# sriram-0311/MC-SLAM

Measured on AMD Instinct MI355X. Metric: multi-cam frames/sec (4-cam 1280x720 @2000 kpts/cam, extract + intra-rig match), higher is better.
Workload: dtype u8; 1 GPU; 4-cam rig 1280x720, 2000 kpts/cam, extract + all-pairs intra-rig match (configs[1]); slots=4, frames_per_launch=128, cameras=4, nfeatures=2000

## Files before the change

### mc-slam_amd/csrc/mcorb_kernels.hip

```cpp
#include <hip/hip_runtime.h>
#include <stdint.h>
#include <string.h>
#include <vector>

#include "mcorb_common.h"
#include "mcorb_device.h"
#include "mcorb_kernels.h"

namespace mcorb {

constexpr int kResizeRows = kResizeTileH;

template <int NF>
__global__ __launch_bounds__(256) void k_resize(uint8_t *__restrict__ pyr, Geom g, int level,
                                                const ResizeTap *__restrict__ tabs, int srcPitch, int srcRows)
{
    extern __shared__ __attribute__((aligned(16))) uint8_t win[];
    const LevelGeom &D = g.lv[level];
    const LevelGeom &S = g.lv[level - 1];
    const int img = blockIdx.z;
    uint8_t *base = pyr + (size_t)img * g.imgBytes;
    const int tid = threadIdx.x;
    const int bx0 = blockIdx.x * 256, by0 = blockIdx.y * kResizeRows;
    const int bx1 = min(bx0 + 255, D.w - 1), by1 = min(by0 + kResizeRows - 1, D.h - 1);
    const int sx0 = tabs[D.xtab + bx0].s0 & ~15, sx1 = tabs[D.xtab + bx1].s1;
    const int sy0 = tabs[D.ytab + by0].s0, sy1 = tabs[D.ytab + by1].s1;
    const int nq = ((sx1 - sx0) >> 4) + 1, nr = sy1 - sy0 + 1;
    const int wave = wave_uniform(tid >> 6);
    const int wy0 = by0 + wave * (kResizeRows / 4);
    uint2 ytap;
    {
        const int l = tid & 63;
        const int dy = min(wy0 + (l < kResizeRows / 4 ? l : 0), D.h - 1);
        ytap = *reinterpret_cast<const uint2 *>(tabs + D.ytab + dy);
    }
    const int dx4 = bx0 + (tid & 63) * 4;
    const int dxc = min(dx4, ((D.w + 3) & ~3) - 4);
    const uint4 t01 = *reinterpret_cast<const uint4 *>(tabs + D.xtab + dxc);
    const uint4 t23 = *reinterpret_cast<const uint4 *>(tabs + D.xtab + dxc + 2);
    {
        const uint8_t *sp = base + S.off + (size_t)sy0 * S.pitch + sx0;
        uint4 *w128 = reinterpret_cast<uint4 *>(win);
        const int pq = srcPitch >> 4;
        const float rcp_pq = 1.0f / (float)pq;
        if constexpr (NF > 0) {
            uint4 v[NF];
            bool ok[NF];
#pragma unroll
            for (int k = 0; k < NF; k++) {
                const int i = tid + 256 * k, ic = min(i, nr * pq - 1);
                const int r = (int)(((float)ic + 0.5f) * rcp_pq), q = ic - r * pq;
                ok[k] = i < nr * pq && q < nq;
                v[k] = *reinterpret_cast<const uint4 *>(sp + (size_t)r * S.pitch + 16 * min(q, nq - 1));
            }
            const int spare = (srcPitch >> 4) * srcRows;
#pragma unroll
            for (int k = 0; k < NF; k++) w128[ok[k] ? tid + 256 * k : spare] = v[k];
        } else {
            for (int i = tid; i < nr * pq; i += 256) {
                const int r = (int)(((float)i + 0.5f) * rcp_pq), q = i - r * pq;
                if (q < nq) w128[i] = *reinterpret_cast<const uint4 *>(sp + (size_t)r * S.pitch + 16 * q);
            }
        }
    }
    __syncthreads();
    asm volatile("" ::"v"(ytap.x), "v"(ytap.y), "v"(t01.x), "v"(t01.y), "v"(t01.z), "v"(t01.w), "v"(t23.x), "v"(t23.y), "v"(t23.z), "v"(t23.w));
    if (dx4 >= D.w) return;
    const uint32_t tw[8] = {t01.x, t01.y, t01.z, t01.w, t23.x, t23.y, t23.z, t23.w};
    int s0[4], s1[4], a0[4], a1[4];
#pragma unroll
    for (int k = 0; k < 4; k++) {
        s0[k] = (int)(tw[2 * k] & 0xffff) - sx0;
        s1[k] = (int)(tw[2 * k] >> 16) - sx0;
        a0[k] = (int)(short)(tw[2 * k + 1] & 0xffff);
        a1[k] = (int)(short)(tw[2 * k + 1] >> 16);
    }
    const uint32_t mask = dx4 + 4 > D.w ? 0xffffffffu >> (8 * (dx4 + 4 - D.w)) : 0xffffffffu;
    int rowA = -1, rowB = -1;
    uint32_t HA[4], HB[4];
    const uint32_t ldsWin = (uint32_t)(uintptr_t)(__attribute__((address_space(3))) void *)win;
    uint32_t sb[4];
#pragma unroll
    for (int k = 0; k < 4; k++) sb[k] = ldsWin + (uint32_t)s0[k];
    auto hrow = [&](int sr, uint32_t *Hout) {
        const uint32_t ro = (uint32_t)__mul24(sr - sy0, srcPitch);
        const uint32_t ad0 = sb[0] + ro, ad1 = sb[1] + ro, ad2 = sb[2] + ro, ad3 = sb[3] + ro;
        uint32_t x0, x1, x2, x3, x4, x5, x6, x7;
        asm volatile("ds_read_u8 %0, %8\n\tds_read_u8 %1, %8 offset:1\n\t"
                     "ds_read_u8 %2, %9\n\tds_read_u8 %3, %9 offset:1\n\t"
                     "ds_read_u8 %4, %10\n\tds_read_u8 %5, %10 offset:1\n\t"
                     "ds_read_u8 %6, %11\n\tds_read_u8 %7, %11 offset:1\n\t"
                     "s_waitcnt lgkmcnt(0)"
                     : "=&v"(x0), "=&v"(x1), "=&v"(x2), "=&v"(x3), "=&v"(x4), "=&v"(x5), "=&v"(x6), "=&v"(x7)
                     : "v"(ad0), "v"(ad1), "v"(ad2), "v"(ad3)
                     : "memory");
        Hout[0] = (__umul24(x0, (uint32_t)a0[0]) + __umul24(x1, (uint32_t)a1[0])) >> 4;
        Hout[1] = (__umul24(x2, (uint32_t)a0[1]) + __umul24(x3, (uint32_t)a1[1])) >> 4;
        Hout[2] = (__umul24(x4, (uint32_t)a0[2]) + __umul24(x5, (uint32_t)a1[2])) >> 4;
        Hout[3] = (__umul24(x6, (uint32_t)a0[3]) + __umul24(x7, (uint32_t)a1[3])) >> 4;
    };
#pragma unroll
    for (int rr = 0; rr < kResizeRows / 4; rr++) {
        const int dy = wy0 + rr;
        if (dy >= D.h) break;
        const uint32_t ys = (uint32_t)__builtin_amdgcn_readlane((int)ytap.x, rr), yc = (uint32_t)__builtin_amdgcn_readlane((int)ytap.y, rr);
        const int r0 = (int)(ys & 0xffff), r1 = (int)(ys >> 16);
        if (r0 != rowA) {
            if (r0 == rowB) {
#pragma unroll
                for (int k = 0; k < 4; k++) HA[k] = HB[k];
            } else {
                hrow(r0, HA);
            }
            rowA = r0;
        }
        if (r1 != rowB) {
            if (r1 == rowA) {
#pragma unroll
                for (int k = 0; k < 4; k++) HB[k] = HA[k];
            } else {
                hrow(r1, HB);
            }
            rowB = r1;
        }
        const uint32_t b0 = yc & 0xffff, b1 = yc >> 16;
        uint32_t p0[4], p1[4];
#pragma unroll
        for (int k = 0; k < 4; k++) {
            p0[k] = __umul24(b0, HA[k]) + 0x20000u;
            p1[k] = __umul24(b1, HB[k]);
        }
        uint32_t t01v, t23v;
        asm("v_add_u32_sdwa %0, %1, %2 dst_sel:DWORD dst_unused:UNUSED_PAD src0_sel:WORD_1 src1_sel:WORD_1" : "=v"(t01v) : "v"(p0[0]), "v"(p1[0]));
        asm("v_add_u32_sdwa %0, %1, %2 dst_sel:WORD_1 dst_unused:UNUSED_PRESERVE src0_sel:WORD_1 src1_sel:WORD_1" : "+v"(t01v) : "v"(p0[1]), "v"(p1[1]));
        asm("v_add_u32_sdwa %0, %1, %2 dst_sel:DWORD dst_unused:UNUSED_PAD src0_sel:WORD_1 src1_sel:WORD_1" : "=v"(t23v) : "v"(p0[2]), "v"(p1[2]));
        asm("v_add_u32_sdwa %0, %1, %2 dst_sel:WORD_1 dst_unused:UNUSED_PRESERVE src0_sel:WORD_1 src1_sel:WORD_1" : "+v"(t23v) : "v"(p0[3]), "v"(p1[3]));
        const u16x2 s01 = __builtin_bit_cast(u16x2, t01v) >> (unsigned short)2, s23 = __builtin_bit_cast(u16x2, t23v) >> (unsigned short)2;
        const uint32_t out = __builtin_amdgcn_perm(__builtin_bit_cast(uint32_t, s23), __builtin_bit_cast(uint32_t, s01), 0x06040200u);
        *reinterpret_cast<uint32_t *>(base + D.off + (size_t)dy * D.pitch + dx4) = out & mask;
    }
}


struct FastCell {
    int on;
    int cell;
    int ph;
    int wi, hi;
    int rows;
    int g0, ng;
    int R;
    float rcp_ng;
    uint32_t headMask, tailMask;
    uint32_t org;
    const uint8_t *src;
    int pitch;
};

constexpr int kFastCellRecDw = 8;
__device__ __forceinline__ void fast_cell_setup(const uint8_t *pyr, const Geom &g, int img, int cell, const uint32_t *__restrict__ rec, FastCell &C)
{
    const uint4 r = *reinterpret_cast<const uint4 *>(rec + (size_t)cell * kFastCellRecDw);
    const uint2 r4 = *reinterpret_cast<const uint2 *>(rec + (size_t)cell * kFastCellRecDw + 4);
    C.cell = cell;
    C.src = pyr + (size_t)img * g.imgBytes + r.x;
    C.org = r.y;
    C.pitch = (int)r.z;
    C.rows = (int)(r.w & 0xff);
    C.wi = (int)((r.w >> 8) & 0xff);
    C.hi = (int)((r.w >> 16) & 0xff);
    C.on = (int)((r.w >> 24) & 1);
    C.ph = (int)((r.w >> 25) & 3);
    C.g0 = (int)(r4.x & 0xff);
    C.ng = (int)((r4.x >> 8) & 0xff);
    C.R = (int)(r4.x >> 16);
    C.rcp_ng = __uint_as_float(r4.y);
    const uint2 r6 = *reinterpret_cast<const uint2 *>(rec + (size_t)cell * kFastCellRecDw + 6);
    C.headMask = r6.x;
    C.tailMask = r6.y;
}

int fast_cell_table(const Geom &g, std::vector<uint32_t> &tab)
{
    const int off = (int)tab.size();
    tab.resize(tab.size() + (size_t)g.cells * kFastCellRecDw, 0u);
    for (int level = 0; level < g.nlevels; level++) {
        const LevelGeom &L = g.lv[level];
        for (int cl = 0; cl < L.nCols * L.nRows; cl++) {
            const int ci = cl / L.nCols, cj = cl - ci * L.nCols;
            const int iniY = kMinBorder + ci * L.hCell;
            int maxY = iniY + L.hCell + 6;
            const int iniX = kMinBorder + cj * L.wCell;
            int maxX = iniX + L.wCell + 6;
            const bool skip = (iniY >= L.maxBorderY - 3) || (iniX >= L.maxBorderX - 6);
            if (maxY > L.maxBorderY) maxY = L.maxBorderY;
            if (maxX > L.maxBorderX) maxX = L.maxBorderX;
            const int cols = maxX - iniX, rows = maxY - iniY;
            const int wi = cols - 6, hi = rows - 6;
            const int ph = iniX & 3, g0 = (ph + 3) >> 2;
            const bool on = !(skip || wi <= 0 || hi <= 0);
            const int ng = on ? ((ph + 2 + wi) >> 2) - g0 + 1 : 1;
            uint32_t *r = tab.data() + off + (size_t)(L.cell0 + cl) * kFastCellRecDw;
            r[0] = on ? (uint32_t)(L.off + (size_t)iniY * L.pitch + (iniX - ph)) : 0u;
            r[1] = ((uint32_t)(ci * L.hCell) << 20) + ((uint32_t)(cj * L.wCell - ph) << 8);
            r[2] = (uint32_t)L.pitch;
            r[3] = on ? ((uint32_t)rows | ((uint32_t)wi << 8) | ((uint32_t)hi << 16) | (1u << 24) | ((uint32_t)ph << 25)) : 0u;
            r[4] = (uint32_t)g0 | ((uint32_t)ng << 8) | ((uint32_t)(64 / ng) << 16);
            const float rcp = 1.0f / (float)ng;
            uint32_t bits;
            memcpy(&bits, &rcp, 4);
            r[5] = bits;
            auto pxmask = [&](int G) {
                static const uint32_t bit[4] = {1u << 15, 1u, 1u << 31, 1u << 16};
                uint32_t m = 0;
                for (int j = 0; j < 4; j++) {
                    const int x = 4 * G + j - (ph + 3);
                    if (x >= 0 && x < wi) m |= bit[j];
                }
                return m;
            };
            r[6] = on ? pxmask(g0) : 0u;
            r[7] = on ? pxmask(g0 + ng - 1) : 0u;
        }
    }
    return off;
}

constexpr int kFastListCap = 768;

#define EMAX __builtin_elementwise_max
#define EMIN __builtin_elementwise_min
struct FastLane {
    int off0;
    uint32_t vmask;
};
template <int TP>
__device__ __forceinline__ FastLane fast_lane_setup(const FastCell &C, int lane)
{
    FastLane L;
    const int r = (int)(((float)lane + 0.5f) * C.rcp_ng);
    const int gi = lane - r * C.ng;
    const bool act = r < C.R;
    L.off0 = act ? (3 + r) * TP + 4 * (C.g0 + gi) : 3 * TP + 4 * C.g0;
    uint32_t m = 0x80018001u;
    m = gi == 0 ? m & C.headMask : m;
    m = gi == C.ng - 1 ? m & C.tailMask : m;
    L.vmask = act ? m : 0u;
    return L;
}

template <int TP>
__device__ __forceinline__ int fast_pass1(const uint8_t *tile, uint32_t *glist, const FastCell &C, int T, int lane, int &row0, int gcap,
                                          const FastLane &L)
{
    const u16x2 Tev = u16x2{(unsigned short)T, (unsigned short)T};
    const u16x2 Tod = u16x2{(unsigned short)(256 * T + 255), (unsigned short)(256 * T + 255)};
    int nG = 0;
    auto trip = [&](int rb, bool tail) {
        int off = L.off0 + rb * TP;
        bool in = true;
        if (tail) {
            in = (int)(((float)lane + 0.5f) * C.rcp_ng) + rb < C.hi;
            off = in ? off : 3 * TP + 4 * C.g0;
        }
        const uint32_t *p = reinterpret_cast<const uint32_t *>(tile + off);
        const uint32_t Cc = p[0], Cl = p[-1], Cr = p[1], Up = p[-3 * (TP / 4)], Dn = p[3 * (TP / 4)];
        const uint32_t Lf = __builtin_amdgcn_alignbyte(Cc, Cl, 1);
        const uint32_t Rt = __builtin_amdgcn_alignbyte(Cr, Cc, 3);
#define U16(X) __builtin_bit_cast(u16x2, (uint32_t)(X))
#define S16(X) __builtin_bit_cast(s16x2, (uint32_t)(X))
        const u16x2 hO = EMIN(EMAX(U16(Up), U16(Dn)), EMAX(U16(Lf), U16(Rt)));
        const u16x2 lO = EMAX(EMIN(U16(Up), U16(Dn)), EMIN(U16(Lf), U16(Rt)));
        const u16x2 hOm = U16(__builtin_bit_cast(uint32_t, hO) & 0xff00ff00u), lOm = U16(__builtin_bit_cast(uint32_t, lO) & 0xff00ff00u);
        const u16x2 vO = U16(Cc & 0xff00ff00u);
        const u16x2 wO = EMAX(__builtin_elementwise_sub_sat(hOm, vO), __builtin_elementwise_sub_sat(vO, lOm));
        const uint32_t zO = __builtin_bit_cast(uint32_t, __builtin_elementwise_sub_sat(wO, Tod));
        const s16x2 vE = S16(Cc & 0x00ff00ffu), uE = S16(Up & 0x00ff00ffu), dE = S16(Dn & 0x00ff00ffu);
        const s16x2 lE = S16(Lf & 0x00ff00ffu), rE = S16(Rt & 0x00ff00ffu);
        const s16x2 wE = EMAX(EMIN(EMAX(uE, dE), EMAX(lE, rE)) - vE, vE - EMAX(EMIN(uE, dE), EMIN(lE, rE)));
        const uint32_t sE = __builtin_bit_cast(uint32_t, __builtin_bit_cast(s16x2, Tev) - wE);
#undef U16
#undef S16
        const uint32_t M = ((sE & 0x80008000u) | (zO & 0x00010001u)) & L.vmask;
        const bool c = M != 0 && in;
        const unsigned long long b = __builtin_amdgcn_ballot_w64(c);
        if (c) glist[lane_rank(b, nG)] = M | ((uint32_t)off >> 1);
        nG += __popcll(b);
    };
    int rb = row0;
    for (; rb + C.R <= C.hi && nG + 64 <= gcap; rb += C.R) trip(rb, false);
    if (rb < C.hi && rb + C.R > C.hi && nG + 64 <= gcap) {
        trip(rb, true);
        rb += C.R;
    }
    row0 = rb;
    return nG;
}

__device__ __forceinline__ int fast_expand(const uint32_t *glist, uint16_t *work, int nG, int lane)
{
    int nA = 0;
    for (int i0 = 0; i0 < nG; i0 += 64) {
        const bool in = i0 + lane < nG;
        const uint32_t E = in ? glist[i0 + lane] : 0u;
        const uint32_t m = E & 0x80018001u;
        const int n1 = in ? __popc(m) - 1 : 0;
        const unsigned long long b0 = __builtin_amdgcn_ballot_w64((n1 & 1) != 0), b1 = __builtin_amdgcn_ballot_w64(n1 >= 2);
        int o = nA + lane + lane_rank(b0) + 2 * lane_rank(b1);
        const uint32_t off = (E & 0x3ffeu) << 1;
        asm volatile("" ::: "memory");
        if (m & 0x8000u) work[o++] = (uint16_t)off;
        if (m & 0x1u) work[o++] = (uint16_t)(off + 1);
        if (m & 0x80000000u) work[o++] = (uint16_t)(off + 2);
        if (m & 0x10000u) work[o++] = (uint16_t)(off + 3);
        const int cnt = min(nG - i0, 64);
        nA += cnt + __popcll(b0) + 2 * __popcll(b1);
        asm volatile("" ::: "memory");
    }
    return nA;
}

template <int TP>
__device__ __forceinline__ int fast_arc_score(const uint8_t *tile, int pos)
{
    int lo = pos - (3 * TP + 3);
    asm volatile("" : "+v"(lo));
    const uint8_t *c = tile + lo + (3 * TP + 3);
    u16x2 X[8];
    X[0] = u16x2{c[3 * TP], c[-3 * TP]};          X[1] = u16x2{c[3 * TP + 1], c[-3 * TP - 1]};
    X[2] = u16x2{c[2 * TP + 2], c[-2 * TP - 2]};  X[3] = u16x2{c[TP + 3], c[-TP - 3]};
    X[4] = u16x2{c[3], c[-3]};                    X[5] = u16x2{c[-TP + 3], c[TP - 3]};
    X[6] = u16x2{c[-2 * TP + 2], c[2 * TP - 2]};  X[7] = u16x2{c[-3 * TP + 1], c[3 * TP - 1]};
    const uint32_t v = c[0];
    u16x2 Sn[8], Sx[8], Pn[8], Px[8];
    Sn[7] = Sx[7] = X[7];
    Pn[0] = Px[0] = X[0];
#pragma unroll
    for (int i = 6; i >= 1; i--) { Sn[i] = EMIN(X[i], Sn[i + 1]); Sx[i] = EMAX(X[i], Sx[i + 1]); }
#pragma unroll
    for (int i = 1; i < 8; i++) { Pn[i] = EMIN(X[i], Pn[i - 1]); Px[i] = EMAX(X[i], Px[i - 1]); }
    Sn[0] = Pn[7]; Sx[0] = Px[7];
    u16x2 bn, bx;
#pragma unroll
    for (int k = 0; k < 8; k++) {
        const u16x2 wn = EMIN(Sn[k], __builtin_shufflevector(Pn[k], Pn[k], 1, 0));
        const u16x2 wx = EMAX(Sx[k], __builtin_shufflevector(Px[k], Px[k], 1, 0));
        bn = k ? EMAX(bn, wn) : wn;
        bx = k ? EMIN(bx, wx) : wx;
    }
    const int Mx = max((int)bn.x, (int)bn.y), Mn = min((int)bx.x, (int)bx.y);
    const int a = max(Mx - (int)v, (int)v - Mn);
    return a < 0 ? 0 : a;
}
#undef EMAX
#undef EMIN

template <int TP>
__global__ __launch_bounds__(64) void k_fast_cells(const uint8_t *__restrict__ pyr, Geom g, int iniTh, int minTh,
                                                   int tileB, int scB, int cap, const uint32_t *__restrict__ cellRec,
                                                   uint32_t *__restrict__ cell_kp, int *__restrict__ cell_cnt)
{
    extern __shared__ __attribute__((aligned(16))) uint8_t lds[];
    constexpr int NQ = TP / 16;
    uint8_t *tile = lds + 16;
    uint8_t *sc = tile + tileB + 16;
    uint8_t *sc2 = sc - 2 * TP;
    uint16_t *work = reinterpret_cast<uint16_t *>(sc + scB + 16);
    uint32_t *glist = reinterpret_cast<uint32_t *>(work + cap / 2);
    const int gcap = cap >> 2;
    struct __attribute__((packed, aligned(4))) Chunk { uint32_t a, b, c, d; };

    const int lane = threadIdx.x;
    const int img = blockIdx.y;
    FastCell C;
    fast_cell_setup(pyr, g, img, wave_uniform(xcd_remap(blockIdx.x, gridDim.x)), cellRec, C);
    int *out_cnt = cell_cnt + (size_t)img * g.cells + C.cell;
    if (!C.on) {
        if (lane == 0) *out_cnt = 0;
        return;
    }

    FastLane FL;
    for (int r = lane; r < C.rows; r += 64) {
        Chunk ch[NQ];
#pragma unroll
        for (int q = 0; q < NQ; q++) ch[q] = *reinterpret_cast<const Chunk *>(C.src + (size_t)r * C.pitch + 16 * q);
        uint4 *dst = reinterpret_cast<uint4 *>(tile + r * TP);
#pragma unroll
        for (int q = 0; q < NQ; q++) dst[q] = uint4{ch[q].a, ch[q].b, ch[q].c, ch[q].d};
    }
    {
        uint4 *s128 = reinterpret_cast<uint4 *>(sc);
        for (int i = lane; i < scB / 16; i += 64) s128[i] = uint4{0, 0, 0, 0};
        FL = fast_lane_setup<TP>(C, lane);
    }
    __syncthreads();

    uint32_t *dst = cell_kp + ((size_t)img * g.cells + C.cell) * g.cellCap;
    int total = 0;
    auto score = [&](int nA, int T) {
        for (int i = lane; i < nA; i += 64) {
            const int pos = work[i];
            const int a = fast_arc_score<TP>(tile, pos);
            sc2[pos] = (uint8_t)(a > T ? a : 0);
        }
    };
    auto nms = [&](int nA) {
        for (int i0 = 0; i0 < nA; i0 += 64) {
            const int i = i0 + lane;
            const int pos = i < nA ? (int)work[i] : 3 * TP;
            int lo = pos - (TP + 1);
            asm volatile("" : "+v"(lo));
            const uint8_t *s = sc2 + lo + (TP + 1);
            const uint32_t a = s[0];
            const uint32_t n = max(max(max((uint32_t)s[1], (uint32_t)s[-1]), max((uint32_t)s[-TP - 1], (uint32_t)s[-TP])),
                                   max(max((uint32_t)s[-TP + 1], (uint32_t)s[TP - 1]), max((uint32_t)s[TP], (uint32_t)s[TP + 1])));
            const bool keep = a > n;
            const unsigned long long b = __builtin_amdgcn_ballot_w64(keep);
            if (keep) {
                const int o = lane_rank(b, total);
                const int yy = (int)(((float)pos + 0.5f) * (1.0f / (float)TP)), xx = __mul24(yy, -TP) + pos;
                if (o < g.cellCap) dst[o] = C.org + ((uint32_t)yy << 20) + ((uint32_t)xx << 8) + (a - 1);
            }
            total += __popcll(b);
        }
    };
    int T = iniTh;
#pragma unroll 1
    for (int attempt = 0; attempt < 2; attempt++) {
        int row0 = 0, sweep = 0;
#pragma unroll 1
        for (;;) {
            const bool whole = row0 == 0;
            const int nG = fast_pass1<TP>(tile, glist, C, T, lane, row0, gcap, FL);
            __syncthreads();
            const int nA = fast_expand(glist, work, nG, lane);
            __syncthreads();
            if (sweep == 0) {
                score(nA, T);
                __syncthreads();
            }
            if (sweep == 1 || (whole && row0 >= C.hi)) nms(nA);
            if (row0 >= C.hi) {
                if (sweep == 1 || whole) break;
                sweep = 1;
                row0 = 0;
            }
            __syncthreads();
        }
        if (total || T == minTh) break;
        T = minTh;
        __syncthreads();
    }
    if (lane == 0) *out_cnt = total;
}

constexpr int kCompactCopies = 4;
template <int kCompactWaves>
__device__ __forceinline__ int block_exclusive_scan(int v, int *wsum, int *total)
{
    const int lane = threadIdx.x & 63, wave = threadIdx.x >> 6;
    int s = v;
#pragma unroll
    for (int o = 1; o < 64; o <<= 1) {
        const int t = __shfl_up(s, o);
        if (lane >= o) s += t;
    }
    if (lane == 63) wsum[wave] = s;
    __syncthreads();
    if (wave == 0) {
        const int w = lane < kCompactWaves ? wsum[lane] : 0;
        int t = w;
#pragma unroll
        for (int o = 1; o < kCompactWaves; o <<= 1) {
            const int u = __shfl_up(t, o);
            if (lane >= o) t += u;
        }
        if (lane < kCompactWaves) wsum[lane] = t - w;
        if (lane == kCompactWaves - 1) *total = t;
    }
    __syncthreads();
    return wsum[wave] + s - v;
}

template <int kCompactWG, int kCompactCells, int NC>
__global__ __launch_bounds__(kCompactWG, 8) void k_compact(const uint32_t *__restrict__ cell_kp, const int *__restrict__ cell_cnt,
                                                        Geom g, const uint16_t *__restrict__ lut, uint32_t *__restrict__ sorted_dev,
                                                        uint32_t *__restrict__ cand, int *__restrict__ tbl,
                                                        int *__restrict__ overflow, int bktCap, int cellsCap)
{
    extern __shared__ __attribute__((aligned(16))) int sh[];
    int *hist = sh;
    uint32_t *bkey = reinterpret_cast<uint32_t *>(hist + NC * bktCap);
    uint16_t *cnts = reinterpret_cast<uint16_t *>(hist + 2 * NC * bktCap);
    constexpr int kCompactWaves = kCompactWG / 64;
    __shared__ int wsum[kCompactWaves];
    __shared__ int s_tot, s_base, s_nz;
    const int tid = threadIdx.x, lane = tid & 63, wave = tid >> 6;
    const int level = blockIdx.y, img = blockIdx.x;
    const LevelGeom &L = g.lv[level];
    const int nc = L.nCols * L.nRows;
    const int *cnt = cell_cnt + (size_t)img * g.cells;
    const int cap = g.cellCap;
    const int B = L.nBuckets;
    const int W0 = L.maxBorderX - kMinBorder, H0 = L.maxBorderY - kMinBorder;
    uint16_t *tx = cnts + cellsCap, *ty = tx + W0;

    int s = 0, t = 0, over = 0;
    for (int c = tid; c < L.cell0; c += kCompactWG) { const int v = cnt[c]; s += v < cap ? v : cap; }
    for (int c = tid; c < nc; c += kCompactWG) {
        int v = cnt[L.cell0 + c];
        if (v > cap) { v = cap; over = 1; }
        cnts[c] = (uint16_t)v;
        t += v;
    }
    for (int c = nc + tid; c < min(nc + 2 * kCompactCells, cellsCap); c += kCompactWG) cnts[c] = 0;
    for (int i = tid; i < W0 + H0; i += kCompactWG) tx[i] = lut[L.lutx + i];
    (void)block_exclusive_scan<kCompactWaves>(s, wsum, &s_base);
    (void)block_exclusive_scan<kCompactWaves>(t, wsum, &s_tot);
    const int base = s_base, T = s_tot;
    for (int b = tid; b < NC * (B + 1); b += kCompactWG) { hist[b] = 0; bkey[b] = 0; }
    int *tb = tbl + (size_t)img * tbl_ints(g.bucketTotal);
    if (tid == 0) {
        s_nz = 0;
        tb[kTblLvlOff + level] = base;
        if (level == g.nlevels - 1) tb[kTblLvlOff + g.nlevels] = base + T;
        if (base + T > g.candCap) over = 1;
    }
    if (over) atomicOr(overflow, 1);
    __syncthreads();

    const uint32_t *src = cell_kp + ((size_t)img * g.cells + L.cell0) * cap;
    const int wave_u = wave_uniform(wave);
    auto walk = [&](auto &&fn) {
        static_assert(kCompactCells == 8 || kCompactCells == 4 || kCompactCells == 2, "the counts are read as one 4-, 8- or 16-byte word");
        constexpr int step = kCompactWaves * kCompactCells;
        const int ncUp = (nc + kCompactCells - 1) & ~(kCompactCells - 1);
        auto load = [&](int c0, int *n, uint32_t *p) {
            if constexpr (kCompactCells == 8) {
                const uint4 q = *reinterpret_cast<const uint4 *>(cnts + c0);
                n[0] = q.x & 0xffff; n[1] = q.x >> 16; n[2] = q.y & 0xffff; n[3] = q.y >> 16;
                n[4] = q.z & 0xffff; n[5] = q.z >> 16; n[6] = q.w & 0xffff; n[7] = q.w >> 16;
            } else if constexpr (kCompactCells == 4) {
                const uint2 q = *reinterpret_cast<const uint2 *>(cnts + c0);
                n[0] = q.x & 0xffff; n[1] = q.x >> 16; n[2] = q.y & 0xffff; n[3] = q.y >> 16;
            } else {
                const uint32_t q = *reinterpret_cast<const uint32_t *>(cnts + c0);
                n[0] = q & 0xffff; n[1] = q >> 16;
            }
#pragma unroll
            for (int u = 0; u < kCompactCells; u++) {
                const uint32_t *cb = src + (size_t)min(c0 + u, nc - 1) * cap;
                p[u] = cb[min(lane, max(n[u], 1) - 1)];
            }
        };
        auto run = [&](int c0, const int *n, const uint32_t *p) {
            int big = 0;
#pragma unroll
            for (int u = 0; u < kCompactCells; u++) {
                big |= n[u];
                if (lane < n[u]) fn(p[u], (c0 + u) * cap + lane);
            }
            if (big > 64) {
#pragma unroll
                for (int u = 0; u < kCompactCells; u++)
                    for (int k = lane + 64; k < n[u]; k += 64) fn(src[(size_t)(c0 + u) * cap + k], (c0 + u) * cap + k);
            }
        };
        int c0 = wave_u * kCompactCells;
        if (c0 >= nc) return;
        int nA[kCompactCells], nB[kCompactCells];
        uint32_t pA[kCompactCells], pB[kCompactCells];
        load(c0, nA, pA);
        while (true) {
            load(min(c0 + step, ncUp), nB, pB);
            run(c0, nA, pA);
            c0 += step;
            if (c0 >= nc) break;
            load(min(c0 + step, ncUp), nA, pA);
            run(c0, nB, pB);
            c0 += step;
            if (c0 >= nc) break;
        }
    };
    walk([&](uint32_t p, int order) {
        const uint32_t code = (uint32_t)tx[cand_x(p)] | (uint32_t)ty[cand_y(p)];
        const uint32_t key = ((uint32_t)cand_resp(p) << 23) | (uint32_t)(kPickOrderMask - order);
        const int slot = (int)code * NC + (lane & (NC - 1));
        atomicAdd(&hist[slot], 1);
        atomicMax(&bkey[slot], key);
    });
    __syncthreads();
    {
        const int bper = (B + kCompactWG - 1) / kCompactWG;
        const int b0 = tid * bper;
        int bs = 0, nzl = 0;
        for (int k = 0; k < bper; k++)
            if (b0 + k < B) {
                int v = 0;
#pragma unroll
                for (int c = 0; c < NC; c++) v += hist[(b0 + k) * NC + c];
                bs += v;
                nzl += v > 0;
            }
        if (nzl) atomicAdd(&s_nz, nzl);
        int brun = block_exclusive_scan<kCompactWaves>(bs, wsum, &s_tot);
        for (int k = 0; k < bper; k++) {
            if (b0 + k < B) {
#pragma unroll
                for (int c = 0; c < NC; c++) { const int v = hist[(b0 + k) * NC + c]; hist[(b0 + k) * NC + c] = brun; brun += v; }
            }
        }
        if (tid == 0) hist[B * NC] = T;
    }
    __syncthreads();
    int *bs_out = tb + kTblHead + L.bucket0;
    for (int b = tid; b <= B; b += kCompactWG) bs_out[b] = hist[b * NC];
    __syncthreads();
    uint32_t *sd = sorted_dev + (size_t)img * g.candCap + base;
    const int room = g.candCap - base;
    walk([&](uint32_t p, int) {
        const uint32_t code = (uint32_t)tx[cand_x(p)] | (uint32_t)ty[cand_y(p)];
        const int slot = atomicAdd(&hist[(int)code * NC + (lane & (NC - 1))], 1);
        if (slot < room) sd[slot] = p;
    });
    __syncthreads();
    uint2 *bb_out = reinterpret_cast<uint2 *>(tb + tbl_win_off(g.bucketTotal)) + L.bucket0;
    for (int b = tid; b < B; b += kCompactWG) {
        uint32_t k = 0;
#pragma unroll
        for (int c = 0; c < NC; c++) k = max(k, bkey[b * NC + c]);
        bb_out[b] = uint2{k, k ? src[kPickOrderMask - (k & (uint32_t)kPickOrderMask)] : 0u};
    }
    bool ship = s_nz < L.quota;
    if (ship && base + T > g.hostCandCap) {
        ship = false;
        if (tid == 0) atomicOr(overflow, 1);
    }
    if (tid == 0) tb[kTblShipped + level] = ship ? 1 : 0;
    if (ship) {
        uint32_t *dst = cand + (size_t)img * g.hostCandCap + base;
        for (int i = tid; i < T; i += kCompactWG) dst[i] = sd[i];
    }
}

template <int B>
__device__ __forceinline__ uint32_t gauss_window(const uint32_t (&D)[4])
{
    constexpr int q = B >> 2, sh = B & 3;
    if constexpr (sh == 0) return D[q];
    else return __builtin_amdgcn_alignbyte(D[q + 1], D[q], sh);
}
template <int SH>
__device__ __forceinline__ void gauss_hsum4(const uint32_t (&D)[4], uint32_t (&h)[4])
{
    constexpr uint32_t T1 = 0x38302212u, T2 = 0x00122230u;
    h[0] = __builtin_amdgcn_udot4(gauss_window<SH + 4>(D), T2, __builtin_amdgcn_udot4(gauss_window<SH>(D), T1, 0u, false), false);
    h[1] = __builtin_amdgcn_udot4(gauss_window<SH + 5>(D), T2, __builtin_amdgcn_udot4(gauss_window<SH + 1>(D), T1, 0u, false), false);
    h[2] = __builtin_amdgcn_udot4(gauss_window<SH + 6>(D), T2, __builtin_amdgcn_udot4(gauss_window<SH + 2>(D), T1, 0u, false), false);
    h[3] = __builtin_amdgcn_udot4(gauss_window<SH + 7>(D), T2, __builtin_amdgcn_udot4(gauss_window<SH + 3>(D), T1, 0u, false), false);
}
__device__ __forceinline__ uint4 gauss_pair4(const uint32_t (&h0)[4], const uint32_t (&h1)[4])
{
    return uint4{__builtin_amdgcn_perm(h1[0], h0[0], 0x05040100u), __builtin_amdgcn_perm(h1[1], h0[1], 0x05040100u),
                 __builtin_amdgcn_perm(h1[2], h0[2], 0x05040100u), __builtin_amdgcn_perm(h1[3], h0[3], 0x05040100u)};
}
__device__ __forceinline__ uint32_t gauss_vrow4(const uint32_t (&P)[5][4], int k)
{
    const int tap[9] = {0, 18, 34, 48, 56, 48, 34, 18, 0};
    const int q = k >> 1, o = 1 - (k & 1);
    uint32_t acc[4];
#pragma unroll
    for (int j = 0; j < 4; j++) {
        uint32_t a = 32768u;
#pragma unroll
        for (int i = 0; i < 4; i++)
            a = __builtin_amdgcn_udot2(__builtin_bit_cast(u16x2, P[q + i][j]), u16x2{(unsigned short)tap[2 * i + o], (unsigned short)tap[2 * i + o + 1]}, a, false);
        acc[j] = a;
    }
    return __builtin_amdgcn_perm(acc[1], acc[0], 0x0c0c0602u) | __builtin_amdgcn_perm(acc[3], acc[2], 0x06020c0cu);
}

__global__ __launch_bounds__(256) void k_blur(const uint8_t *__restrict__ pyr, uint8_t *__restrict__ blur, Geom g)
{
    constexpr int TW = kBlurTW, TH = kBlurTH;
    constexpr int ID = TW / 4 + 8, A0 = 3;
    constexpr int NP = (TH + 6) / 2;
    __shared__ __attribute__((aligned(16))) uint32_t in32[(TH + 6) * ID];
    __shared__ __attribute__((aligned(16))) uint32_t hp[NP * TW];
    const int tid = threadIdx.x;
    const int img = blockIdx.y;
    const int tile = xcd_remap(blockIdx.x, gridDim.x);
    int level = 0;
#pragma unroll 1
    for (int l = 1; l < g.nlevels; l++)
        if (tile >= g.lv[l].tile0) level = l;
    const LevelGeom &L = g.lv[level];
    const int t = tile - L.tile0;
    const int ty = t / L.tilesX, tx = t - ty * L.tilesX;
    const int x0 = tx * TW, y0 = ty * TH;
    const uint8_t *plane = pyr + (size_t)img * g.imgBytes + L.off;

    if (x0 >= 4 && x0 + TW + 4 <= L.w && y0 >= 3 && y0 + TH + 3 <= L.h) {
        constexpr int QR = TW / 16;
        constexpr int NQ = ((TH + 6) * QR + 255) / 256;
        const uint8_t *src = plane + (size_t)(y0 - 3) * L.pitch + x0;
        uint4 v[NQ];
#pragma unroll
        for (int k = 0; k < NQ; k++) {
            const int i = tid + 256 * k;
            const int r = i / QR, q = i - r * QR;
            v[k] = i < (TH + 6) * QR ? *reinterpret_cast<const uint4 *>(src + (size_t)r * L.pitch + 16 * q) : uint4{0, 0, 0, 0};
        }
        uint32_t ap = 0;
        const int ar = tid >> 1, aside = tid & 1;
        if (tid < 2 * (TH + 6)) ap = *reinterpret_cast<const uint32_t *>(src + (size_t)ar * L.pitch + (aside ? TW : -4));
#pragma unroll
        for (int k = 0; k < NQ; k++) {
            const int i = tid + 256 * k;
            const int r = i / QR, q = i - r * QR;
            if (i < (TH + 6) * QR) *reinterpret_cast<uint4 *>(in32 + r * ID + A0 + 1 + 4 * q) = v[k];
        }
        if (tid < 2 * (TH + 6)) in32[ar * ID + A0 + (aside ? TW / 4 + 1 : 0)] = ap;
    } else {
        constexpr int QR = TW / 16;
        constexpr int NQ = ((TH + 6) * QR + 255) / 256;
        auto src_row = [&](int r) {
            int sy = reflect101(y0 + r - 3, L.h);
            sy = sy < 0 ? 0 : (sy >= L.h ? L.h - 1 : sy);
            return plane + (size_t)sy * L.pitch + x0;
        };
        uint4 v[NQ];
#pragma unroll
        for (int k = 0; k < NQ; k++) {
            const int i = tid + 256 * k;
            const int r = i / QR, q = i - r * QR;
            v[k] = i < (TH + 6) * QR ? *reinterpret_cast<const uint4 *>(src_row(r) + 16 * q) : uint4{0, 0, 0, 0};
        }
        uint32_t ap = 0;
        const int ar = tid >> 1, aside = tid & 1;
        if (tid < 2 * (TH + 6) && (aside || x0 > 0)) ap = *reinterpret_cast<const uint32_t *>(src_row(ar) + (aside ? TW : -4));
#pragma unroll
        for (int k = 0; k < NQ; k++) {
            const int i = tid + 256 * k;
            const int r = i / QR, q = i - r * QR;
// ... 730 lines not shown
```

Measured before the change: 40490 frames/s.

## Rework FAST cell kernel with raw LDS addressing, score-map reuse and corner compaction

```diff
diff --git a/mc-slam_amd/csrc/mcorb_kernels.hip b/mc-slam_amd/csrc/mcorb_kernels.hip
--- a/mc-slam_amd/csrc/mcorb_kernels.hip
+++ b/mc-slam_amd/csrc/mcorb_kernels.hip
@@ -231,40 +231,57 @@
 #define EMAX __builtin_elementwise_max
 #define EMIN __builtin_elementwise_min
 struct FastLane {
-    int off0;
+    uint32_t G0;
     uint32_t vmask;
+    int r;
 };
+typedef __attribute__((address_space(3))) uint8_t lds_byte;
+__device__ __forceinline__ uint32_t lds_addr(const void *p) { return (uint32_t)(uintptr_t)(const lds_byte *)p; }
+template <typename T>
+__device__ __forceinline__ T lds_ld(uint32_t a) { return *(const __attribute__((address_space(3))) T *)(uintptr_t)a; }
+template <typename T>
+__device__ __forceinline__ void lds_st(uint32_t a, T v) { *(__attribute__((address_space(3))) T *)(uintptr_t)a = v; }
+
 template <int TP>
-__device__ __forceinline__ FastLane fast_lane_setup(const FastCell &C, int lane)
+__device__ __forceinline__ FastLane fast_lane_setup(const FastCell &C, int lane, uint32_t tileA)
 {
     FastLane L;
     const int r = (int)(((float)lane + 0.5f) * C.rcp_ng);
     const int gi = lane - r * C.ng;
     const bool act = r < C.R;
-    L.off0 = act ? (3 + r) * TP + 4 * (C.g0 + gi) : 3 * TP + 4 * C.g0;
+    L.G0 = tileA - 4 + (act ? r * TP + 4 * (C.g0 + gi) : 4 * C.g0);
     uint32_t m = 0x80018001u;
     m = gi == 0 ? m & C.headMask : m;
     m = gi == C.ng - 1 ? m & C.tailMask : m;
     L.vmask = act ? m : 0u;
+    L.r = r;
     return L;
 }
 
-template <int TP>
-__device__ __forceinline__ int fast_pass1(const uint8_t *tile, uint32_t *glist, const FastCell &C, int T, int lane, int &row0, int gcap,
-                                          const FastLane &L)
+template <int TP, bool FROM_MAP>
+__device__ __forceinline__ int fast_pass1(uint32_t tileA, uint32_t glistA, const FastCell &C, int T, int lane, int &row0, int gcap,
+                                          const FastLane &L, uint32_t scD)
 {
     const u16x2 Tev = u16x2{(unsigned short)T, (unsigned short)T};
     const u16x2 Tod = u16x2{(unsigned short)(256 * T + 255), (unsigned short)(256 * T + 255)};
-    int nG = 0;
-    auto trip = [&](int rb, bool tail) {
-        int off = L.off0 + rb * TP;
-        bool in = true;
-        if (tail) {
-            in = (int)(((float)lane + 0.5f) * C.rcp_ng) + rb < C.hi;
-            off = in ? off : 3 * TP + 4 * C.g0;
-        }
-        const uint32_t *p = reinterpret_cast<const uint32_t *>(tile + off);
-        const uint32_t Cc = p[0], Cl = p[-1], Cr = p[1], Up = p[-3 * (TP / 4)], Dn = p[3 * (TP / 4)];
+    uint32_t slot = glistA;
+    const uint32_t slotMax = glistA + 4 * (gcap - 64);
+    auto emit = [&](uint32_t G, uint32_t M, bool in) {
+        const bool c = M != 0 && in;
+        const unsigned long long b = __builtin_amdgcn_ballot_w64(c);
+        asm volatile("" : "+s"(slot));
+        if (c) lds_st<uint32_t>(slot + 4 * lane_rank(b), M | G);
+        slot += 4 * __popcll(b);
+    };
+    auto trip = [&](uint32_t G, bool in) {
+        if constexpr (FROM_MAP) {
+            const uint32_t sc4 = lds_ld<uint32_t>(G + scD);
+            const uint32_t nz = ((sc4 & 0x7f7f7f7fu) + 0x7f7f7f7fu) | sc4;
+            emit(G, (((nz & 0x00800080u) << 8) | ((nz >> 15) & 0x00010001u)) & L.vmask, in);
+            return;
+        }
+        const uint32_t Up = lds_ld<uint32_t>(G + 4), Dn = lds_ld<uint32_t>(G + 6 * TP + 4);
+        const uint32_t Cl = lds_ld<uint32_t>(G + 3 * TP), Cc = lds_ld<uint32_t>(G + 3 * TP + 4), Cr = lds_ld<uint32_t>(G + 3 * TP + 8);
         const uint32_t Lf = __builtin_amdgcn_alignbyte(Cc, Cl, 1);
         const uint32_t Rt = __builtin_amdgcn_alignbyte(Cr, Cc, 3);
 #define U16(X) __builtin_bit_cast(u16x2, (uint32_t)(X))
@@ -281,38 +298,43 @@
         const uint32_t sE = __builtin_bit_cast(uint32_t, __builtin_bit_cast(s16x2, Tev) - wE);
 #undef U16
 #undef S16
-        const uint32_t M = ((sE & 0x80008000u) | (zO & 0x00010001u)) & L.vmask;
-        const bool c = M != 0 && in;
-        const unsigned long long b = __builtin_amdgcn_ballot_w64(c);
-        if (c) glist[lane_rank(b, nG)] = M | ((uint32_t)off >> 1);
-        nG += __popcll(b);
+        uint32_t sel = (sE & 0x80008000u) | (zO & ~0x80008000u);
+        asm volatile("" : "+v"(sel));
+        emit(G, sel & L.vmask, in);
     };
     int rb = row0;
-    for (; rb + C.R <= C.hi && nG + 64 <= gcap; rb += C.R) trip(rb, false);
-    if (rb < C.hi && rb + C.R > C.hi && nG + 64 <= gcap) {
-        trip(rb, true);
+    uint32_t G = L.G0 + rb * TP;
+    for (; rb + C.R <= C.hi && slot <= slotMax; rb += C.R, G += C.R * TP) {
+        asm volatile("" : "+v"(G));
+        trip(G, true);
+    }
+    if (rb < C.hi && rb + C.R > C.hi && slot <= slotMax) {
+        const bool in = L.r + rb < C.hi;
+        uint32_t Gt = in ? G : tileA - 4 + 4 * C.g0;
+        asm volatile("" : "+v"(Gt));
+        trip(Gt, in);
         rb += C.R;
     }
     row0 = rb;
-    return nG;
-}
-
-__device__ __forceinline__ int fast_expand(const uint32_t *glist, uint16_t *work, int nG, int lane)
+    return (int)(slot - glistA) >> 2;
+}
+
+__device__ __forceinline__ int fast_expand(uint32_t glistA, uint32_t workA, int nG, int lane)
 {
     int nA = 0;
     for (int i0 = 0; i0 < nG; i0 += 64) {
         const bool in = i0 + lane < nG;
-        const uint32_t E = in ? glist[i0 + lane] : 0u;
+        const uint32_t E = in ? lds_ld<uint32_t>(glistA + 4 * (i0 + lane)) : 0u;
         const uint32_t m = E & 0x80018001u;
         const int n1 = in ? __popc(m) - 1 : 0;
         const unsigned long long b0 = __builtin_amdgcn_ballot_w64((n1 & 1) != 0), b1 = __builtin_amdgcn_ballot_w64(n1 >= 2);
-        int o = nA + lane + lane_rank(b0) + 2 * lane_rank(b1);
-        const uint32_t off = (E & 0x3ffeu) << 1;
+        uint32_t o = (workA + 2 * nA) + 2 * (lane_rank(b0, lane) + 2 * lane_rank(b1));
+        const uint32_t G = E & 0x7ffcu;
         asm volatile("" ::: "memory");
-        if (m & 0x8000u) work[o++] = (uint16_t)off;
-        if (m & 0x1u) work[o++] = (uint16_t)(off + 1);
-        if (m & 0x80000000u) work[o++] = (uint16_t)(off + 2);
-        if (m & 0x10000u) work[o++] = (uint16_t)(off + 3);
+        if ((int16_t)E < 0) { lds_st<uint16_t>(o, (uint16_t)G); o += 2; }
+        if (m & 0x1u) { lds_st<uint16_t>(o, (uint16_t)(G + 1)); o += 2; }
+        if (m & 0x80000000u) { lds_st<uint16_t>(o, (uint16_t)(G + 2)); o += 2; }
+        if (m & 0x10000u) lds_st<uint16_t>(o, (uint16_t)(G + 3));
         const int cnt = min(nG - i0, 64);
         nA += cnt + __popcll(b0) + 2 * __popcll(b1);
         asm volatile("" ::: "memory");
@@ -321,17 +343,15 @@
 }
 
 template <int TP>
-__device__ __forceinline__ int fast_arc_score(const uint8_t *tile, int pos)
-{
-    int lo = pos - (3 * TP + 3);
-    asm volatile("" : "+v"(lo));
-    const uint8_t *c = tile + lo + (3 * TP + 3);
+__device__ __forceinline__ int fast_arc_score(uint32_t W)
+{
+    auto px = [&](int dx, int dy) { return (unsigned short)lds_ld<uint8_t>(W + 1 + (3 + dy) * TP + (3 + dx)); };
     u16x2 X[8];
-    X[0] = u16x2{c[3 * TP], c[-3 * TP]};          X[1] = u16x2{c[3 * TP + 1], c[-3 * TP - 1]};
-    X[2] = u16x2{c[2 * TP + 2], c[-2 * TP - 2]};  X[3] = u16x2{c[TP + 3], c[-TP - 3]};
-    X[4] = u16x2{c[3], c[-3]};                    X[5] = u16x2{c[-TP + 3], c[TP - 3]};
-    X[6] = u16x2{c[-2 * TP + 2], c[2 * TP - 2]};  X[7] = u16x2{c[-3 * TP + 1], c[3 * TP - 1]};
-    const uint32_t v = c[0];
+    X[0] = u16x2{px(0, 3), px(0, -3)};   X[1] = u16x2{px(1, 3), px(-1, -3)};
+    X[2] = u16x2{px(2, 2), px(-2, -2)};  X[3] = u16x2{px(3, 1), px(-3, -1)};
+    X[4] = u16x2{px(3, 0), px(-3, 0)};   X[5] = u16x2{px(3, -1), px(-3, 1)};
+    X[6] = u16x2{px(2, -2), px(-2, 2)};  X[7] = u16x2{px(1, -3), px(-1, 3)};
+    const uint32_t v = px(0, 0);
     u16x2 Sn[8], Sx[8], Pn[8], Px[8];
     Sn[7] = Sx[7] = X[7];
     Pn[0] = Px[0] = X[0];
@@ -364,9 +384,10 @@
     constexpr int NQ = TP / 16;
     uint8_t *tile = lds + 16;
     uint8_t *sc = tile + tileB + 16;
-    uint8_t *sc2 = sc - 2 * TP;
-    uint16_t *work = reinterpret_cast<uint16_t *>(sc + scB + 16);
-    uint32_t *glist = reinterpret_cast<uint32_t *>(work + cap / 2);
+    const uint32_t tileA = lds_addr(tile);
+    const uint32_t scD = (uint32_t)tileB + TP + 20;
+    const uint32_t workA = tileA + tileB + 16 + scB + 16;
+    const uint32_t glistA = workA + cap;
     const int gcap = cap >> 2;
     struct __attribute__((packed, aligned(4))) Chunk { uint32_t a, b, c, d; };
 
@@ -392,35 +413,54 @@
     {
         uint4 *s128 = reinterpret_cast<uint4 *>(sc);
         for (int i = lane; i < scB / 16; i += 64) s128[i] = uint4{0, 0, 0, 0};
-        FL = fast_lane_setup<TP>(C, lane);
+        FL = fast_lane_setup<TP>(C, lane, tileA);
     }
     __syncthreads();
 
     uint32_t *dst = cell_kp + ((size_t)img * g.cells + C.cell) * g.cellCap;
     int total = 0;
-    auto score = [&](int nA, int T) {
-        for (int i = lane; i < nA; i += 64) {
-            const int pos = work[i];
-            const int a = fast_arc_score<TP>(tile, pos);
-            sc2[pos] = (uint8_t)(a > T ? a : 0);
-        }
+    const int posK = 3 * TP + 4 - (int)tileA;
+    const uint32_t orgW = C.org + ((uint32_t)posK << 8);
+    const float rowK = (float)posK + 0.5f;
+    auto score = [&](int nA, int T, bool compact) {
+        int nC = 0;
+        for (int i0 = 0; i0 < nA; i0 += 64) {
+            const int i = i0 + lane;
+            uint32_t W = 0;
+            bool corner = false;
+            if (i < nA) {
+                W = lds_ld<uint16_t>(workA + 2 * i);
+                const int a = fast_arc_score<TP>(W);
+                corner = a > T;
+                lds_st<uint8_t>(W + scD, (uint8_t)(corner ? a : 0));
+            }
+            asm volatile("" ::: "memory");
+            if (compact) {
+                const unsigned long long b = __builtin_amdgcn_ballot_w64(corner);
+                uint32_t slot0 = workA + 2 * nC;
+                asm volatile("" : "+s"(slot0));
+                if (corner) lds_st<uint16_t>(slot0 + 2 * lane_rank(b), (uint16_t)W);
+                nC += __popcll(b);
+            }
+            asm volatile("" ::: "memory");
+        }
+        return nC;
     };
     auto nms = [&](int nA) {
         for (int i0 = 0; i0 < nA; i0 += 64) {
             const int i = i0 + lane;
-            const int pos = i < nA ? (int)work[i] : 3 * TP;
-            int lo = pos - (TP + 1);
-            asm volatile("" : "+v"(lo));
-            const uint8_t *s = sc2 + lo + (TP + 1);
-            const uint32_t a = s[0];
-            const uint32_t n = max(max(max((uint32_t)s[1], (uint32_t)s[-1]), max((uint32_t)s[-TP - 1], (uint32_t)s[-TP])),
-                                   max(max((uint32_t)s[-TP + 1], (uint32_t)s[TP - 1]), max((uint32_t)s[TP], (uint32_t)s[TP + 1])));
+            const uint32_t W = i < nA ? (uint32_t)lds_ld<uint16_t>(workA + 2 * i) : tileA - 4;
+            const uint32_t S = W + (scD - (TP + 1));
+            auto sc8 = [&](int dx, int dy) { return (uint32_t)lds_ld<uint8_t>(S + (1 + dy) * TP + (1 + dx)); };
+            const uint32_t a = sc8(0, 0);
+            const uint32_t n = max(max(max(sc8(1, 0), sc8(-1, 0)), max(sc8(-1, -1), sc8(0, -1))),
+                                   max(max(sc8(1, -1), sc8(-1, 1)), max(sc8(0, 1), sc8(1, 1))));
             const bool keep = a > n;
             const unsigned long long b = __builtin_amdgcn_ballot_w64(keep);
             if (keep) {
-                const int o = lane_rank(b, total);
-                const int yy = (int)(((float)pos + 0.5f) * (1.0f / (float)TP)), xx = __mul24(yy, -TP) + pos;
-                if (o < g.cellCap) dst[o] = C.org + ((uint32_t)yy << 20) + ((uint32_t)xx << 8) + (a - 1);
+                const uint32_t o = lane_rank(b);
+                const int yy = (int)(((float)W + rowK) * (1.0f / (float)TP)), xw = __mul24(yy, -TP) + (int)W;
+                if ((int)o < g.cellCap - total) (dst + total)[o] = orgW + ((uint32_t)yy << 20) + ((uint32_t)xw << 8) + (a - 1);
             }
             total += __popcll(b);
         }
@@ -432,15 +472,18 @@
 #pragma unroll 1
         for (;;) {
             const bool whole = row0 == 0;
-            const int nG = fast_pass1<TP>(tile, glist, C, T, lane, row0, gcap, FL);
+            const int nG = sweep == 0 ? fast_pass1<TP, false>(tileA, glistA, C, T, lane, row0, gcap, FL, scD)
+                                      : fast_pass1<TP, true>(tileA, glistA, C, T, lane, row0, gcap, FL, scD);
             __syncthreads();
-            const int nA = fast_expand(glist, work, nG, lane);
+            int nA = fast_expand(glistA, workA, nG, lane);
             __syncthreads();
+            const bool last = sweep == 1 || (whole && row0 >= C.hi);
             if (sweep == 0) {
-                score(nA, T);
+                const int nC = score(nA, T, last);
+                nA = last ? nC : nA;
                 __syncthreads();
             }
-            if (sweep == 1 || (whole && row0 >= C.hi)) nms(nA);
+            if (last) nms(nA);
             if (row0 >= C.hi) {
                 if (sweep == 1 || whole) break;
                 sweep = 1;
```

Measured after the change: 41260 frames/s, median of 5. +1.9%, better.
